# unlikeghost/DeepLearning-MPI

Hardware: AMD Instinct MI355X
Metric: images/sec (whole node) ResNet-50 DDP bs=256/GPU (higher is better)
Workload: dtype bf16; 1 GPU; model=resnet50, global_batch=256, image=224, in_channels=3, per_gpu_batch=256, parallelism=dp1, backend=single, device=cuda, optimizer=SGD(momentum=0.9, wd=1e-5), hipgraph=False

## Files before the change

### deeplearning_mpi_amd/csrc/binding/conv_bwd.cpp

```cpp
#include <c10/hip/HIPCachingAllocator.h>

#include <algorithm>
#include <vector>

#include "common.h"
#include "ops.h"

namespace dlmpi_ext {

using dlmpi::ConvArgs;
using dlmpi::ConvPhase;
using dlmpi::DgradStreamArgs;
using dlmpi::make_fastdiv;
using dlmpi::WgradArgs;

c10::optional<at::Tensor> conv2d_dgrad_pro(const at::Tensor& dy, int N, int P, int Q, int K, int lddy, int dyoff,
                                       const at::Tensor& wT, int C, int R, int S, int stride, int pad, int H, int W,
                                       at::Tensor dx, int lddx, int dxoff, const c10::optional<at::Tensor>& res,
                                       int ldres, int resoff, const c10::optional<at::Tensor>& mask, int ldmask,
                                       int maskoff, const c10::optional<at::Tensor>& z, int ldz, int zoff,
                                       const c10::optional<at::Tensor>& z2, int ldz2, int z2off,
                                       const c10::optional<at::Tensor>& mscale,
                                       const c10::optional<at::Tensor>& mshift,
                                       const c10::optional<at::Tensor>& mbits, bool colsum, int pro,
                                       const c10::optional<at::Tensor>& pk0, const c10::optional<at::Tensor>& pk1,
                                       const c10::optional<at::Tensor>& pz, int ldpz, int pzoff,
                                       const c10::optional<at::Tensor>& bias) {
  require_gpu(dy, "dy");
  if (stride > 2) throw std::runtime_error("conv2d_dgrad: stride <= 2 supported");
  if (bias.has_value() && bias->defined() && (bias->scalar_type() != at::kFloat || bias->numel() < C))
    throw std::runtime_error("conv2d_dgrad: bias must be fp32 [C]");
  ConvArgs a{};
  a.f32 = act_f32(dy, "conv2d_dgrad");
  same_type(dy, wT, "conv2d_dgrad wT");
  same_type(dy, dx, "conv2d_dgrad dx");
  same_type(dy, res, "conv2d_dgrad res");
  same_type(dy, mask, "conv2d_dgrad mask");
  same_type(dy, z, "conv2d_dgrad z");
  same_type(dy, z2, "conv2d_dgrad z2");
  a.x = ptr<uint16_t>(dy);
  a.H = P; a.W = Q; a.C = K; a.ldx = lddy; a.xoff = dyoff;
  a.w = ptr<uint16_t>(wT);
  a.ldw = R * S * K;
  a.S = S;
  a.OH = H; a.OW = W;
  a.so = stride; a.sa = 1;
  a.Nimg = N; a.Kout = C;
  fill_epilogue(a, dx, lddx, dxoff, bias, res, ldres, resoff, c10::nullopt, c10::nullopt, false, c10::nullopt);
  a.vec_store = ((lddx % 8) == 0 && (dxoff % 8) == 0) ? 1 : 0;
  a.mask = optr<uint16_t>(mask);
  a.ldmask = ldmask; a.maskoff = maskoff;
  a.z = optr<uint16_t>(z);
  a.ldz = ldz; a.zoff = zoff;
  a.z2 = optr<uint16_t>(z2);
  a.ldz2 = ldz2; a.z2off = z2off;
  a.mscale = optr<float>(mscale);
  a.mshift = optr<float>(mshift);
  a.mbits = optr<uint8_t>(mbits);
  if (a.mbits && (mbits->numel() != (int64_t)N * H * W * (C / 8) || C % 8))
    throw std::runtime_error("conv2d_dgrad: mask bits must be [N*H*W][C/8]");
  a.nstat = a.z2 ? 3 : 2;
  if (a.z && !a.mask && !a.mscale && !a.mbits)
    throw std::runtime_error("conv2d_dgrad: fused BN statistics need the ReLU mask");
  if (a.mscale && (!a.z || !a.mshift)) throw std::runtime_error("conv2d_dgrad: mask from z needs z, scale, shift");
  if ((a.mask || a.mscale || a.mbits) && ((ldmask | maskoff | ldz | zoff | ldz2 | z2off) % 8 != 0 || !a.vec_store))
    throw std::runtime_error("conv2d_dgrad: fused BN tensors must be 8-channel aligned");
  g_ran.dgrad_stream = 0;
  g_ran.conv3 = 0;
  if (R == 1 && S == 1 && K == 8) g_ran.head_dgrad = 0;
  {
    const int mode = a.mscale ? 2 : 0;
    int th, tw, G;
    if (stream3x3_shape(N, H, W, K, C, R, S, stride, pad, pro, a.f32, th, tw, G) && P == H && Q == W && !colsum &&
        !a.mask && !a.mbits && !a.z2 && !a.res && !a.bias && (a.z != nullptr) == (mode == 2) && a.vec_store &&
        a.kvalid == C && (lddy | dyoff) % 8 == 0 && (int64_t)H * W * lddx * 2 < (1ll << 31) &&
        dx.scalar_type() == at::kBFloat16) {
      dlmpi::Conv3StreamArgs c = conv3_args(dy, N, H, W, lddy, dyoff, wT, 1, a.y, lddx, dxoff, th, tw, G);
      c.z = static_cast<const uint16_t*>(a.z);
      c.ldz = ldz; c.zoff = zoff;
      c.mscale = a.mscale; c.mshift = a.mshift;
      c10::optional<at::Tensor> st;
      if (a.z) {
        st = at::empty({(int64_t)G, 2, (int64_t)C}, dy.options().dtype(at::kFloat));
        c.stats = ptr<float>(*st);
      }
      check(dlmpi_conv3x3_stream(&c, mode == 2 ? 2 : 1, cur_stream()), "conv2d_dgrad (stream 3x3)");
      g_ran.conv3 = 1;
      return st;
    }
  }
  {
    const int64_t M = (int64_t)N * H * W;
    const int mode = a.mbits ? 1 : (a.mscale ? 2 : 0);
    int sbm, sbn, G;
    const auto fits = [](int64_t rows, int64_t ld) { return rows * ld < (1ll << 31); };
    if (R == 1 && S == 1 && stride == 1 && pad == 0 && !a.f32 && pro == 0 && !colsum && !a.mask &&
        (a.z != nullptr) == (mode != 0) && a.vec_store && a.kvalid == C && (lddy | dyoff) % 8 == 0 &&
        (!a.res || (ldres | resoff) % 8 == 0) && fits(M, lddy) && fits(M, lddx) && (!a.res || fits(M, ldres)) &&
        (!a.z || fits(M, ldz)) && (!a.z2 || fits(M, ldz2)) && dx.scalar_type() == at::kBFloat16 &&
        dlmpi_dgrad_stream_plan(M, K, C, mode, a.z2 ? 1 : 0, a.res ? 1 : 0, &sbm, &sbn, &G)) {
      DgradStreamArgs sa{};
      sa.x = ptr<uint16_t>(dy);
      sa.ldx = lddy; sa.xoff = dyoff;
      sa.w = ptr<uint16_t>(wT);
      sa.y = reinterpret_cast<uint16_t*>(a.y);
      sa.ldy = lddx; sa.yoff = dxoff;
      sa.y_bytes = (int)std::min<int64_t>(INT32_MAX, (int64_t)dx.numel() * 2);
      sa.M = (int)M; sa.K = K; sa.Kout = C;
      sa.bias = a.bias;
      sa.res = static_cast<const uint16_t*>(a.res);
      sa.ldres = ldres; sa.resoff = resoff;
      sa.z = static_cast<const uint16_t*>(a.z);
      sa.ldz = ldz; sa.zoff = zoff;
      sa.z2 = static_cast<const uint16_t*>(a.z2);
      sa.ldz2 = ldz2; sa.z2off = z2off;
      sa.mbits = a.mbits;
      sa.mscale = a.mscale; sa.mshift = a.mshift;
      sa.G = G; sa.ntiles = C / sbn; sa.mtiles = (int)ceil_div(M, sbm);
      c10::optional<at::Tensor> st;
      if (a.z) {
        st = at::empty({(int64_t)G, (int64_t)a.nstat, (int64_t)C}, dy.options().dtype(at::kFloat));
        sa.stats = ptr<float>(*st);
// ... 229 lines not shown
  a.ntiles = ceil_div(a.TC, bn);
  const int tiles = a.mtiles * a.ntiles;
  const int target_blocks = g_sw.wgrad_blocks > 0 ? g_sw.wgrad_blocks : 512;
  const int maxsplit = std::max(1, ceil_div(a.npix, 512));
  int splits = std::max(1, std::min(maxsplit, w256 ? target_blocks / tiles : ceil_div(target_blocks, tiles)));
  int pps = ceil_div(a.npix, splits);
  pps = ceil_div(pps, 64) * 64;
  splits = ceil_div(a.npix, pps);
  a.splits = splits;
  a.pix_per_split = pps;
  a.fdPQ = make_fastdiv((uint32_t)(P * Q));
  a.fdQ = make_fastdiv((uint32_t)Q);
  a.fdC = make_fastdiv((uint32_t)C);
  a.fdS = make_fastdiv((uint32_t)S);
  const int64_t wsz = (int64_t)Ko * a.TC;
  const int G = splits > 1 ? dlmpi_wgrad_reduce_groups(splits, wsz) : 0;
  at::Tensor ws = at::empty({(int64_t)(splits + G) * wsz}, dy.options().dtype(at::kFloat));
  a.ws = ptr<float>(ws);
  check(dlmpi_conv_wgrad(&a, bm, bn, cur_stream()), "conv2d_wgrad");
  wgrad_reduce_or_defer(ws, splits, G, wsz, Ko, R * S, C, Creal, Ko_real, grad);
}

void conv2d_wgrad(const at::Tensor& dy, int lddy, int dyoff, int Ko, const at::Tensor& x, int N, int H, int W, int C,
                  int ldx, int xoff, int R, int S, int stride, int pad, int P, int Q, at::Tensor grad, int Creal,
                  int Ko_real) {
  conv2d_wgrad_pro(dy, lddy, dyoff, Ko, x, N, H, W, C, ldx, xoff, R, S, stride, pad, P, Q, grad, Creal, Ko_real, 0,
                   c10::nullopt, c10::nullopt, 0, 0, 0, c10::nullopt, c10::nullopt);
}

void register_conv_bwd(pybind11::module& m) {
  m.def("conv2d_dgrad", &conv2d_dgrad);
  m.def("conv2d_dgrad_pro", &conv2d_dgrad_pro);
  m.def("conv2d_wgrad", &conv2d_wgrad);
  m.def("conv2d_wgrad_pro", &conv2d_wgrad_pro);
  m.def("set_wgrad_defer", [](bool on) {
    if (!on) wgrad_flush();
    g_wgrad_defer = on;
  });
  m.def("wgrad_flush", &wgrad_flush);
  m.def("wgrad_discard", &wgrad_discard);
  m.def("set_wgrad_batch", [](int n) { g_wgrad_batch = n > 0 && n <= dlmpi::kWgradBatch ? n : dlmpi::kWgradBatch; });
  m.def("set_defer_direct", [](int on) { g_defer_direct = on != 0; });
  m.def("set_wgrad_bypass", [](bool on) { g_wgrad_bypass = on; });
  m.def("wgrad_pending", []() { return (int)g_pending.size(); });
  m.def("wgrad_reduce_launches", []() { return g_reduce_launches; });
  m.def("set_dgrad_stream", [](int mode) { dlmpi_set_dgrad_stream(mode); });
  m.def("set_wgrad_fast", [](int on) { dlmpi_set_wgrad_fast(on); });
  def_int(m, "set_conv_pipe_dgrad", nullptr, &g_sw.pipe_dgrad);
  def_int(m, "set_wgrad3", nullptr, &g_sw.wgrad3);
  def_int(m, nullptr, "wgrad3_last", &g_ran.wgrad3);
  def_int(m, "set_wgrad3_blocks", nullptr, &g_sw.wgrad3_blocks);
  def_int(m, "set_wgrad_blocks", nullptr, &g_sw.wgrad_blocks);
  def_int(m, nullptr, "dgrad_stream_last", &g_ran.dgrad_stream);
  def_int(m, nullptr, "head_dgrad_last", &g_ran.head_dgrad);
}

}
```

### deeplearning_mpi_amd/csrc/binding/conv_plan.h

```cpp
#pragma once
#include <cstdint>
#include <vector>

#include "../kernels/dlmpi_kernels.h"

namespace dlmpi_ext {

static inline int ceil_div(int64_t a, int64_t b) { return (int)((a + b - 1) / b); }

struct Switches {
  int pipe = -1;
  int pipe_dgrad = -1;
  int apply = -1;
  int halo = -1;
  int halo_first = 1;
  int splitk = 0;
  int autotune = -1;
  int head = 1;
  int c8 = 1;
  int c16 = 1;
  int c3pro = 1;
  int convT_stream = 1;
  int wgrad3 = -1;
  int wgrad3_blocks = 0;
  int wgrad_blocks = 0;
};
struct LastRan {
  int halo = 0;
  int stream = 0;
  int dgrad_stream = 0;
  int conv3 = 0;
  int head = 0;
  int c8 = 0;
  int c16 = 0;
  int convT_stream = 0;
  int wgrad3 = 0;
  int head_dgrad = 0;
};
extern Switches g_sw;
extern LastRan g_ran;
bool conv_autotune_on();

struct ConvShape {
  int N, H, W, C, K, R, S, stride, pad;
  int pro, f32;
  int bm_req, bn_req;
  int P() const { return (H + 2 * pad - R) / stride + 1; }
  int Q() const { return (W + 2 * pad - S) / stride + 1; }
  int64_t M() const { return (int64_t)N * P() * Q(); }
  int64_t red() const { return (int64_t)R * S * C; }
  bool free_tiles() const { return bm_req <= 0 && bn_req <= 0; }
};

enum class FwdPath { c8, c16, head, stream3x3, stream1x1, apply1x1, pipe, halo, igemm };
const char* fwd_path_name(FwdPath p);

struct FwdOperands {
  bool has_res, has_scale, relu, has_stats, has_fin;
  int kvalid;
  int ldx, xoff, ldy, yoff, ldw;
  int ldpro;
  bool y_bf16, y_f32, w_bf16;
  bool plain(int K) const { return !has_res && !has_scale && !relu && kvalid == K; }
  bool x_aligned() const { return ldx % 8 == 0 && xoff % 8 == 0; }
  bool y_aligned() const { return ldy % 8 == 0 && yoff % 8 == 0; }
};

struct FwdPlan {
  FwdPath path;
  int bm, bn, pipe;
  int rows;
  int G, th, tw, sbm, sbn;
};

void set_kstep(dlmpi::ConvArgs& a, int C);

struct TileQuery {
  int64_t M;
  int Kout;
  int64_t red;
  int cin;
  int R, S, stride, pad, P, Q;
  int f32, pro;
// ... 25 lines not shown
```

### deeplearning_mpi_amd/csrc/kernels/conv_igemm.hip

```cpp
#include <cstdlib>
#include <type_traits>

#include "common.h"

namespace dlmpi {

typedef __attribute__((address_space(3))) void lds_void;

__device__ __forceinline__ void glds16(const void* g, char* lds_wave_base) {
  __builtin_amdgcn_global_load_lds(g, (lds_void*)lds_wave_base, 16, 0, 0);
}

template <int BM, int BN, int NT, int WM>
struct EpiSmem {
  static constexpr int NP0 = BM < 128 ? 1 : (BM / 64 < WM / 16 ? BM / 64 : WM / 16);
  static constexpr int NP = (WM / 16) % NP0 == 0 ? NP0 : WM / 16;
  static constexpr int CS_LD = BN + 4;
  static constexpr int EPI = (BM / NP) * CS_LD * 4;
  static constexpr int RED = (NT / (BN / 8)) * 3 * BN * 4;
  static constexpr int bytes = EPI > RED ? EPI : RED;
};

template <int NT, int NF>
__device__ __forceinline__ bool splitk_combine(const ConvArgs& a, f32x4* acc, char* smem, int tid, int mt, int nt) {
// ... 872 lines not shown
    issue_halo();
    issue_b(0);
  }
  auto step = [&](int ks, auto SLc) {
    constexpr int sl = decltype(SLc)::value;
    asm volatile("s_waitcnt vmcnt(0)\n\ts_waitcnt lgkmcnt(0)" ::: "memory");
    __builtin_amdgcn_s_barrier();
    asm volatile("" ::: "memory");
    int a_addr[TM];
#pragma unroll
    for (int mi = 0; mi < TM; ++mi) {
      const int r = hb[mi] + toff;
      a_addr[mi] = r * 128 + ((fg ^ (r & 7)) << 4);
    }
    const bool more = ks + 1 < nk;
    const bool chunk_end = more && t_cur + 1 == NTAP;
    if (more) tap_next();
#pragma unroll
    for (int kk = 0; kk < 2; ++kk) {
      const int ch = kk * 4 + fg;
      bf16x8 af[TM], bfr[TN];
#pragma unroll
      for (int ni = 0; ni < TN; ++ni)
        bfr[ni] = *reinterpret_cast<const bf16x8*>(smem + b_row0 + sl * B_BYTES + ni * 16 * 128 + ((ch ^ sw) << 4));
#pragma unroll
      for (int mi = 0; mi < TM; ++mi)
        af[mi] = *reinterpret_cast<const bf16x8*>(smem + (kk ? (a_addr[mi] ^ 64) : a_addr[mi]));
      if (kk == 0 && more && !chunk_end) {
        issue_b(sl ^ 1);
        asm volatile("" ::: "memory");
      }
#pragma unroll
      for (int mi = 0; mi < TM; ++mi)
#pragma unroll
        for (int ni = 0; ni < TN; ++ni)
          acc[mi][ni] = __builtin_amdgcn_mfma_f32_16x16x32_bf16(af[mi], bfr[ni], acc[mi][ni], 0, 0, 0);
    }
    if (chunk_end) {
      asm volatile("s_waitcnt lgkmcnt(0)" ::: "memory");
      __builtin_amdgcn_s_barrier();
      asm volatile("" ::: "memory");
      issue_halo();
      issue_b(sl ^ 1);
    }
  };
  for (int ks = 0; ks < nk; ks += 2) {
    step(ks, std::integral_constant<int, 0>{});
    if (ks + 1 < nk) step(ks + 1, std::integral_constant<int, 1>{});
  }
  __syncthreads();
  conv_epilogue<BM, BN, NT, WGM, WGN, uint16_t, true>(a, ph, acc, smem, tid, m0, n0, mt, hn, hh0, hw0);
}

template <int BM, int BN, int WGM, int WGN>
__global__ __launch_bounds__(512) __attribute__((amdgpu_waves_per_eu(BN <= 128 ? 4 : 2, 8)))
void conv1x1_apply_kernel(const ConvArgs a) {
  constexpr int NT = 512;
  static_assert(WGM * WGN == 8, "8 waves");
  constexpr int WM = BM / WGM, WN = BN / WGN, TM = WM / 16, TN = WN / 16;
  constexpr int A_BYTES = BM * 128, B_BYTES = BN * 128, SB = A_BYTES + B_BYTES;
  constexpr int MAXC = 4 * BN;
  constexpr int PRM_BYTES = 4 * MAXC * 4;
  constexpr int EPI_NEED = EpiSmem<BM, BN, NT, WM>::bytes;
  constexpr int SMEM = 2 * SB + PRM_BYTES > EPI_NEED ? 2 * SB + PRM_BYTES : EPI_NEED;
  constexpr int RP = NT / 8;
  constexpr int AL = BM / RP, BL = BN / RP;
  static_assert(AL >= 1 && BL >= 1, "tile shape");
  __shared__ __attribute__((aligned(16))) char smem[SMEM];

  const int tid = threadIdx.x, lane = tid & 63;
  const int wid = __builtin_amdgcn_readfirstlane(tid >> 6);
  const int wm = wid / WGN, wn = wid % WGN;
  const int lrow = tid >> 3, jc = tid & 7;
  const ConvPhase& ph = a.ph[0];
  const int M = a.Nimg * ph.P * ph.Q;
  const uint32_t mt = xcd_remap(blockIdx.x, (uint32_t)ph.mtiles);
  const int m0 = (int)mt * BM;
  const int C = a.C, nk = C / 64;
  const bool rbn = a.prscale != nullptr;

  float* prm = reinterpret_cast<float*>(smem + 2 * SB);
  for (int i = tid; i < C; i += NT) {
    prm[i] = a.pscale[i];
    prm[MAXC + i] = a.pshift[i];
    if (rbn) {
      prm[2 * MAXC + i] = a.prscale[i];
      prm[3 * MAXC + i] = a.prshift[i];
    }
  }

  const uint16_t* xb = static_cast<const uint16_t*>(a.x);
  const uint16_t* rb = static_cast<const uint16_t*>(a.pz);
  uint32_t zo[AL], ro[AL], yo[AL], bo[AL];
  uint32_t okm = 0;
#pragma unroll
  for (int i = 0; i < AL; ++i) {
    const int m = m0 + lrow + RP * i;
    if (m < M) okm |= 1u << i;
    const uint32_t mm = m < M ? (uint32_t)m : 0u;
    zo[i] = mm * (uint32_t)a.ldx + (uint32_t)a.xoff + 8 * jc;
    ro[i] = mm * (uint32_t)a.ldpz + (uint32_t)a.pzoff + 8 * jc;
    yo[i] = mm * (uint32_t)a.ldpy + (uint32_t)a.pyoff + 8 * jc;
    bo[i] = mm * (uint32_t)(C >> 3) + jc;
  }
  const uint16_t* wb = static_cast<const uint16_t*>(a.w) + (int64_t)lrow * a.ldw + 8 * jc;
  const int64_t wstep = (int64_t)RP * a.ldw;

  u32x4 zv[AL], rv[AL], wv[BL];
  auto load = [&](int k) {
    const int c = 64 * k;
#pragma unroll
    for (int i = 0; i < AL; ++i) {
      zv[i] = *reinterpret_cast<const u32x4*>(xb + zo[i] + c);
      rv[i] = *reinterpret_cast<const u32x4*>(rb + ro[i] + c);
    }
#pragma unroll
    for (int i = 0; i < BL; ++i) wv[i] = *reinterpret_cast<const u32x4*>(wb + i * wstep + c);
  };
  auto commit = [&](int k, int buf) {
    char* As = smem + buf * SB;
    char* Bs = As + A_BYTES;
    const int cc = 64 * k + 8 * jc;
    const f32x4 s0 = *reinterpret_cast<const f32x4*>(prm + cc), s1 = *reinterpret_cast<const f32x4*>(prm + cc + 4);
    const f32x4 h0 = *reinterpret_cast<const f32x4*>(prm + MAXC + cc);
    const f32x4 h1 = *reinterpret_cast<const f32x4*>(prm + MAXC + cc + 4);
#pragma unroll
    for (int i = 0; i < AL; ++i) {
      const int r = lrow + RP * i;
      u32x4 pk = u32x4{0u, 0u, 0u, 0u};
      if ((okm >> i) & 1) {
        float v[8], q[8];
        unpack8(zv[i], v);
        unpack8(rv[i], q);
#pragma unroll
        for (int e = 0; e < 4; ++e) {
          v[e] = __builtin_fmaf(v[e], s0[e], h0[e]);
          v[e + 4] = __builtin_fmaf(v[e + 4], s1[e], h1[e]);
        }
        if (rbn) {
          const f32x4 a0 = *reinterpret_cast<const f32x4*>(prm + 2 * MAXC + cc);
          const f32x4 a1 = *reinterpret_cast<const f32x4*>(prm + 2 * MAXC + cc + 4);
          const f32x4 b0 = *reinterpret_cast<const f32x4*>(prm + 3 * MAXC + cc);
          const f32x4 b1 = *reinterpret_cast<const f32x4*>(prm + 3 * MAXC + cc + 4);
#pragma unroll
          for (int e = 0; e < 4; ++e) {
            q[e] = __builtin_fmaf(q[e], a0[e], b0[e]);
            q[e + 4] = __builtin_fmaf(q[e + 4], a1[e], b1[e]);
          }
        }
#pragma unroll
        for (int e = 0; e < 8; ++e) v[e] = fmaxf(v[e] + q[e], 0.f);
        pk = pack8(v);
        *reinterpret_cast<u32x4*>(a.py + yo[i] + 64 * k) = pk;
        uint32_t b = 0;
#pragma unroll
        for (int t = 0; t < 4; ++t) {
          b |= (uint32_t)((pk[t] & 0xffffu) != 0u && !(pk[t] & 0x8000u)) << (2 * t);
          b |= (uint32_t)((pk[t] >> 16) != 0u && !(pk[t] & 0x80000000u)) << (2 * t + 1);
        }
        a.pmbits[bo[i] + 8 * k] = (uint8_t)b;
      }
      *reinterpret_cast<u32x4*>(As + r * 128 + ((jc ^ (r & 7)) << 4)) = pk;
    }
#pragma unroll
    for (int i = 0; i < BL; ++i) {
      const int r = lrow + RP * i;
      *reinterpret_cast<u32x4*>(Bs + r * 128 + ((jc ^ (r & 7)) << 4)) = wv[i];
    }
  };

  f32x4 acc[TM][TN];
#pragma unroll
  for (int mi = 0; mi < TM; ++mi)
#pragma unroll
    for (int ni = 0; ni < TN; ++ni) acc[mi][ni] = f32x4{0.f, 0.f, 0.f, 0.f};
  const int fr = lane & 15, fg = lane >> 4;

  load(0);
  __syncthreads();
  commit(0, 0);
  __syncthreads();
  for (int k = 0; k < nk; ++k) {
    if (k + 1 < nk) load(k + 1);
// ... 47 lines not shown
  return S < 2 ? 1 : S;
}

static hipError_t launch_f32(const ConvArgs* a, int bm, int bn, dim3 grid, hipStream_t s) {
  if (a->pro != 0) return hipErrorInvalidValue;
  const bool small = a->C < 32 || a->C % 32 != 0;
#define LAUNCH_F32(BM_, BN_)                                                                                   \
  do {                                                                                                       \
    if (small) hipLaunchKernelGGL((conv_igemm_kernel<BM_, BN_, true, 2, 0, float>), grid, dim3(256), 0, s, *a); \
    else hipLaunchKernelGGL((conv_igemm_kernel<BM_, BN_, false, 2, 0, float>), grid, dim3(256), 0, s, *a);     \
  } while (0)
  if (bm == 128 && bn == 128) LAUNCH_F32(128, 128);
  else if (bm == 128 && bn == 64) LAUNCH_F32(128, 64);
  else if (bm == 64 && bn == 128) LAUNCH_F32(64, 128);
  else if (bm == 64 && bn == 64) LAUNCH_F32(64, 64);
  else return hipErrorInvalidValue;
#undef LAUNCH_F32
  return hipGetLastError();
}

static hipError_t launch_pipe(const ConvArgs* a, int bm, int bn, int var, dim3 grid, hipStream_t s) {
  if (a->f32 || a->pro != 0 || a->C % 64 != 0 || a->C > kPipeMaxC || a->halo || grid.y != 1) return hipErrorInvalidValue;
  if (var != (bm == 128 ? 4 : 2)) return hipErrorInvalidValue;
  if (bm == 256 && bn == 256) hipLaunchKernelGGL((conv_pipe_kernel<256, 256, 2, 4, 2, 2>), grid, dim3(512), 0, s, *a);
  else if (bm == 224 && bn == 256) hipLaunchKernelGGL((conv_pipe_kernel<224, 256, 2, 4, 2, 2>), grid, dim3(512), 0, s, *a);
  else if (bm == 256 && bn == 128) hipLaunchKernelGGL((conv_pipe_kernel<256, 128, 4, 2, 3, 2>), grid, dim3(512), 0, s, *a);
  else if (bm == 128 && bn == 256) hipLaunchKernelGGL((conv_pipe_kernel<128, 256, 2, 4, 3, 4>), grid, dim3(512), 0, s, *a);
  else if (bm == 512 && bn == 64) hipLaunchKernelGGL((conv_pipe_kernel<512, 64, 8, 1, 2, 2>), grid, dim3(512), 0, s, *a);
  else return hipErrorInvalidValue;
  return hipGetLastError();
}

extern "C" int dlmpi_conv1x1_apply_ok(int C, int K) {
  return C % 64 == 0 && C <= 4 * K && (K == 64 || K == 128 || K == 256);
}

extern "C" hipError_t dlmpi_conv1x1_apply(const ConvArgs* a, int bm, hipStream_t s) {
  if (a->pro != 3 || a->f32 || a->halo || a->nphase != 1 || a->ntiles != 1 || !a->vec_store || a->res ||
      a->scale || a->relu || a->mask || a->mscale || a->mbits || a->z || a->splitk_req > 1 ||
      !dlmpi_conv1x1_apply_ok(a->C, a->Kout) || a->ph[0].Tr != 1 || a->ph[0].Ts != 1 || a->sa != 1 ||
      a->ph[0].mtiles != (a->Nimg * a->ph[0].P * a->ph[0].Q + bm - 1) / bm || a->ldw != a->C ||
      (int64_t)a->Nimg * a->H * a->W * (a->ldx > a->ldpz ? (a->ldx > a->ldpy ? a->ldx : a->ldpy)
                                                          : (a->ldpz > a->ldpy ? a->ldpz : a->ldpy)) >= (1ll << 31))
    return hipErrorInvalidValue;
  const dim3 grid((unsigned)a->ph[0].mtiles);
  if (grid.x == 0) return hipSuccess;
  if (bm == 128 && a->Kout == 64) hipLaunchKernelGGL((conv1x1_apply_kernel<128, 64, 8, 1>), grid, dim3(512), 0, s, *a);
  else if (bm == 128 && a->Kout == 128) hipLaunchKernelGGL((conv1x1_apply_kernel<128, 128, 4, 2>), grid, dim3(512), 0, s, *a);
  else if (bm == 128 && a->Kout == 256) hipLaunchKernelGGL((conv1x1_apply_kernel<128, 256, 2, 4>), grid, dim3(512), 0, s, *a);
  else return hipErrorInvalidValue;
  return hipGetLastError();
}

static int g_halo_pipe = 1;
extern "C" void dlmpi_set_halo_pipe(int on) { g_halo_pipe = on; }

extern "C" hipError_t dlmpi_conv_igemm_ex(const ConvArgs* a_in, int bm, int bn, int pipe, hipStream_t s) {
  int maxt = 0, tiles = 0, maxk = 0;
  for (int i = 0; i < a_in->nphase; ++i) {
    maxt = a_in->ph[i].mtiles > maxt ? a_in->ph[i].mtiles : maxt;
    tiles += a_in->ph[i].mtiles * a_in->ntiles;
    maxk = a_in->ph[i].ksteps > maxk ? a_in->ph[i].ksteps : maxk;
  }
  ConvArgs ab = *a_in;
  const ConvArgs* a = &ab;
  ab.splitk = 1;
  if (pipe) {
    const dim3 grid((unsigned)(maxt * a->ntiles), 1, (unsigned)a->nphase);
    if (grid.x == 0) return hipSuccess;
    return launch_pipe(a, bm, bn, pipe - 1, grid, s);
  }
  int S = a_in->splitk_req > 0 ? a_in->splitk_req : splitk_plan(tiles, maxk);
  if (S > maxk) S = maxk > 0 ? maxk : 1;
  if (S > 1) {
    const int ntile_ids = maxt * a_in->ntiles * a_in->nphase;
    float* slab = dlmpi_splitk_slab(s, (size_t)ntile_ids * S * bm * bn);
    int* tk = dlmpi_splitk_tickets(s, ntile_ids);
    if (slab && tk) {
      ab.splitk = S;
      ab.sk_slab = slab;
      ab.sk_tk = tk;
    }
  }
  dim3 grid((unsigned)(maxt * a->ntiles), (unsigned)ab.splitk, (unsigned)a->nphase);
  if (grid.x == 0) return hipSuccess;
  if (a->f32) return launch_f32(a, bm, bn, grid, s);
  if (a->halo) {
    if (a->pro != 0 || a->C % 64 != 0) return hipErrorInvalidValue;
    if (bm == 128 && bn == 128) hipLaunchKernelGGL((conv_igemm_kernel<128, 128, false, 2, 0, uint16_t, true>), grid, dim3(256), 0, s, *a);
    else if (bm == 128 && bn == 64) hipLaunchKernelGGL((conv_igemm_kernel<128, 64, false, 2, 0, uint16_t, true>), grid, dim3(256), 0, s, *a);
    else if (bm == 256 && bn == 64) hipLaunchKernelGGL((conv_igemm_kernel<256, 64, false, 4, 0, uint16_t, true>), grid, dim3(256), 0, s, *a);
    else if (bm == 256 && bn == 128) {
      if (g_halo_pipe && ab.splitk == 1) hipLaunchKernelGGL((conv_halo_pipe_kernel<256, 128, 2>), grid, dim3(256), 0, s, *a);
      else hipLaunchKernelGGL((conv_igemm_kernel<256, 128, false, 2, 0, uint16_t, true>), grid, dim3(256), 0, s, *a);
    } else return hipErrorInvalidValue;
    return hipGetLastError();
  }
  if (a->pro != 0 && (a->pro != 3 || a->C < 64 || a->C % 64 != 0)) return hipErrorInvalidValue;
  hipError_t e = hipSuccess;
  if (bm == 256 && bn == 64) {
    if (a->pro == 3) return hipErrorInvalidValue;
    if (a->C < 64) hipLaunchKernelGGL((conv_igemm_kernel<256, 64, true, 4>), grid, dim3(256), 0, s, *a);
    else hipLaunchKernelGGL((conv_igemm_kernel<256, 64, false, 4>), grid, dim3(256), 0, s, *a);
  } else if (bm == 256 && bn == 128) e = launch_tile<256, 128>(a, grid, s);
  else if (bm == 128 && bn == 128) e = launch_tile<128, 128>(a, grid, s);
  else if (bm == 128 && bn == 64) e = launch_tile<128, 64>(a, grid, s);
// ... 10 lines not shown
```

### deeplearning_mpi_amd/csrc/kernels/dlmpi_kernels.h

```cpp
#pragma once
#include <hip/hip_runtime_api.h>
#include <stdint.h>

namespace dlmpi {

struct FastDiv {
  uint32_t d, mul, shr;
};
inline FastDiv make_fastdiv(uint32_t d) {
  FastDiv f;
  f.d = d;
  uint32_t l = 0;
  while ((1ull << l) < d) ++l;
  f.mul = (uint32_t)((((1ull << 32) * ((1ull << l) - d)) / d) + 1);
  f.shr = l;
  return f;
}

struct FinArgs {
  int mode;
  double count;
  const float* gamma;
  const float* beta;
  float* running_mean;
// ... 143 lines not shown
  const uint16_t* w;
  int ldw, flip;
  uint16_t* y;
  int ldy, yoff;
  int N, H, W;
  int th, tw, tiles_h, tiles_w, ntiles, G;
  const float* bias;
  const uint16_t* z;
  int ldz, zoff;
  const float* mscale;
  const float* mshift;
  float* stats;
  const float* psc;
  const float* psh;
  uint16_t* py;
  int ldpy, pyoff;
};

struct WgradReduceEntry {
  const float* ws;
  float* ws2;
  float* out;
  int64_t total;
  int splits, G, Ko_real, T, Cpad, Creal;
  int block1;
  int block2;
};
constexpr int kWgradBatch = 16;
struct WgradReduceBatch {
  int n;
  WgradReduceEntry e[kWgradBatch];
};

struct Wgrad3Args {
  const void* dy;
  int ldy, dyoff, Ko;
  const void* x;
  int ldx, xoff, C;
  int H, W;
  int tiles_h, tiles_w, ntiles_pix, tiles_per_split;
  int mtiles, ntiles, splits;
  float* ws;
};

}

extern "C" {
void dlmpi_set_wgrad_fast(int on);
void dlmpi_set_halo_pipe(int on);
hipError_t dlmpi_conv_igemm(const dlmpi::ConvArgs* a, int bm, int bn, hipStream_t s);
hipError_t dlmpi_conv_igemm_ex(const dlmpi::ConvArgs* a, int bm, int bn, int pipe, hipStream_t s);
int dlmpi_conv1x1_apply_ok(int C, int K);
hipError_t dlmpi_conv1x1_apply(const dlmpi::ConvArgs* a, int bm, hipStream_t s);
hipError_t dlmpi_conv_wgrad(const dlmpi::WgradArgs* a, int bm, int bn, hipStream_t s);
int dlmpi_wgrad_pro_ok(int direct, int pro_a, int pro_b);
hipError_t dlmpi_wgrad_reduce(const float* ws, int splits, int Ko, int T, int Cpad, int Creal,
                              int Ko_real, float* out, float* ws2, int ws2_floats, hipStream_t s);
int dlmpi_wgrad_reduce_groups(int splits, int64_t total);
hipError_t dlmpi_wgrad_reduce_batch(dlmpi::WgradReduceBatch* b, hipStream_t s);
int dlmpi_wgrad3_plan(int Ko, int C, int* kt, int* ct);
hipError_t dlmpi_wgrad3x3(const dlmpi::Wgrad3Args* a, int kt, int ct, hipStream_t s);
int dlmpi_head1x1_ok(int C, int kv);
int dlmpi_conv3x3_c8_blocks(int64_t pixels);
int dlmpi_conv4x4_c16_blocks(int64_t pixels);
hipError_t dlmpi_conv4x4_c16(const void* x, int ldx, int xoff, int N, int U, int V, const void* w, const float* bias,
                             void* y, int ldy, int yoff, float* stats, int G, hipStream_t s);
hipError_t dlmpi_conv3x3_c8(const void* x, int ldx, int xoff, int N, int H, int W, const void* w, const float* bias,
                            void* y, int ldy, int yoff, float* stats, int G, hipStream_t s);
hipError_t dlmpi_head1x1(const void* x, int ldx, int xoff, int64_t M, int C, const void* w, int ldw,
                         const float* bias, void* y, int ldy, int yoff, int kv, int y_f32, const float* psc,
                         const float* psh, hipStream_t s);
int dlmpi_conv3_stream_plan(int N, int H, int W, int C, int K, int blocks, int* th, int* tw, int* G);
hipError_t dlmpi_conv3x3_stream(const dlmpi::Conv3StreamArgs* a, int mode, hipStream_t s);
void dlmpi_set_conv3_stream(int mode);

hipError_t dlmpi_bn_finalize(const float* partial, int ntiles, int C, double count, const float* gamma,
                             const float* beta, float* running_mean, float* running_var, float momentum,
                             float eps, float* scale, float* shift, float* save_mean, float* save_invstd,
                             double* ws, hipStream_t s);
int dlmpi_colsum_ws_doubles(int T, int C);
hipError_t dlmpi_set_aux_stream(hipStream_t s, int role);
hipError_t dlmpi_bn_stats(const void* x, int64_t M, int C, int ldx, int xoff, float* partial, int nblk, int f32,
                          hipStream_t s);
hipError_t dlmpi_bn_apply(const void* x, int ldx, int xoff, int64_t M, int C, const float* scale, const float* shift,
                          const void* res, int ldres, int resoff, int relu, void* y, int ldy, int yoff, uint8_t* mbits,
                          int f32, hipStream_t s);
hipError_t dlmpi_bn_apply2(const void* x, int ldx, int xoff, int64_t M, int C, const float* scale, const float* shift,
                           const void* res, int ldres, int resoff, const float* rscale, const float* rshift, int relu,
                           void* y, int ldy, int yoff, uint8_t* mbits, int f32, hipStream_t s);
hipError_t dlmpi_bn_bwd_reduce(const void* dy, int lddy, int dyoff, const void* ymask, int ldym, int ymoff,
                               const void* x, int ldx, int xoff, int64_t M, int C, const float* mean,
                               const float* invstd, float* partial, int nblk, int f32, hipStream_t s);
hipError_t dlmpi_bn_bwd_finalize(const float* partial, int nblk, int C, double count, const float* gamma,
                                 const float* mean, const float* invstd, float* dgamma, float* dbeta,
                                 float* coef, double* ws, hipStream_t s);
hipError_t dlmpi_bn_bwd_finalize_ex(const float* partial, int nblk, int ns, int k2, int raw_z, int C, double count,
                                    const float* gamma, const float* mean, const float* invstd, float* dgamma,
                                    float* dbeta, float* coef, double* ws, hipStream_t s);
hipError_t dlmpi_bn_bwd_apply(const void* dy, int lddy, int dyoff, const void* ymask, int ldym, int ymoff,
                              const void* x, int ldx, int xoff, int64_t M, int C, const float* coef, void* dx,
                              void* dyr_out, int f32, hipStream_t s);
hipError_t dlmpi_dual_dgrad_weights(const void* w, int C, int K, const float* coef, void* w2, float* b, int f32,
                                    hipStream_t s);
hipError_t dlmpi_channel_sum(const void* x, int64_t M, int C, int ldx, int xoff, float* out_acc, float* partial,
                             int nblk, double* ws, int f32, hipStream_t s);
int dlmpi_reduce_blocks(int64_t M, int C);
// ... 102 lines not shown
```

### deeplearning_mpi_amd/models/engine.py

```python
from __future__ import annotations

import contextlib
import os
from typing import NamedTuple, Optional

import torch
import torch.nn as nn

from ..ops.act import Act, Deferred, padc
from ..ops.backend import make_backend
from ..utils.arena import ParamArena
from ..utils.profiler import range as trace_range


@contextlib.contextmanager
def grad_side(be, *tensors):
    side = getattr(be, "side_stream", None)
    if side is None:
        yield
        return
    cur = torch.cuda.current_stream()
    side.wait_stream(cur)
    torch.cuda.set_stream(side)
    try:
        yield
    finally:
        torch.cuda.set_stream(cur)
    if _STREAM_HOLD:
        be.held.extend(t for t in tensors if t is not None)
        return
    for t in tensors:
        if t is not None:
            t.record_stream(side)


def record_on(stream, *objs):
    if _STREAM_HOLD:
        return
    for o in objs:
        if o is None:
            continue
        if isinstance(o, torch.Tensor):
            if o.is_cuda:
                o.record_stream(stream)
        elif isinstance(o, Deferred):
            record_on(stream, *o.bufs())
        elif hasattr(o, "buf") and isinstance(getattr(o, "buf"), torch.Tensor):
            record_on(stream, o.buf)
        elif isinstance(o, (tuple, list)):
            record_on(stream, *o)


_STREAM_HOLD = True

_OUTER_DGRAD = True
_HEAD_DGRAD = True

DEFER_BN_WGRAD = True

DUAL_DGRAD = True
DUAL_MIN_ROWS = 2 * 256 * 28 * 28
DUAL_WGRAD_PRO = True

FUSE_APPLY = True
FUSE_APPLY_MAX_K = 256
FUSE_APPLY_3X3 = True

WGRAD_TAIL_MAIN = True


def img_rows(a, n0: int, n1: int):
    if a is None:
        return None
    if isinstance(a, Deferred):
        return Deferred(a.kind, img_rows(a.src, n0, n1), img_rows(a.z, n0, n1), a.k0, a.k1)
    hw = a.H * a.W
    return Act(a.buf[n0 * hw:n1 * hw], n1 - n0, a.H, a.W, a.C, a.off)


class PendingApply:

    __slots__ = ("y", "z", "scale", "shift", "res", "relu", "mbits", "done")

    def __init__(self, y, z, scale, shift, res, relu, mbits):
        self.y, self.z, self.scale, self.shift, self.res, self.relu, self.mbits = y, z, scale, shift, res, relu, mbits
        self.done = False

    N = property(lambda self: self.y.N)
    H = property(lambda self: self.y.H)
    W = property(lambda self: self.y.W)
    C = property(lambda self: self.y.C)
    device = property(lambda self: self.y.device)

    def resolve(self, be) -> Act:
        if not self.done:
            be.bn_apply(self.z, self.scale, self.shift, self.res, self.relu, self.y, mbits=self.mbits)
            self.done = True
        return self.y


def resolve(be, a):
    return a.resolve(be) if isinstance(a, PendingApply) else a


def bufs(*objs):
    out = []
    for o in objs:
        if o is None:
            continue
        if isinstance(o, Deferred):
            out.extend(o.bufs())
        elif isinstance(o, Act):
            out.append(o.buf)
        else:
            out.append(o)
    return out


class BwdFuse(NamedTuple):
# ... 168 lines not shown
        if before_res is not None and res is not None:
            before_res()
        invstd = torch.rsqrt(bn.running_var + bn.eps)
        scale = bn.weight.data * invstd if bn.affine else invstd
        shift = (bn.bias.data if bn.affine else 0.0) - bn.running_mean * scale
        if self.bias is not None:
            shift = shift + self.bias.data * scale
        be.conv_fwd(x, wf, self.Kp, self.R, self.S, self.stride, self.pad, y, res=res, scale=scale.contiguous(),
                    shift=shift.contiguous(), relu=self.relu)
        return y, None

    @staticmethod
    def fuse_spec(ctx, z2=None) -> BwdFuse:
        x, z, y, mean, invstd, scale, shift, has_res, mbits = ctx
        if has_res or z2 is not None:
            return BwdFuse(None if mbits is not None else y, z, z2, mbits=mbits)
        return BwdFuse(None, z, None, scale, shift)

    def bwd(self, be, ctx, dy: Act, need_dx=True, dx_res: Act = None, dyr_out: Act = None, ymask: Act = None,
            use_own_mask=True, pre=None, k2=1, fuse_next=None, colsum=False, before_res=None, dx_out: Act = None):
        ar = self.arena
        bn = self.bn
        dg_in, dg_w, dg_b = None, None, None
        if bn is not None and need_dx and pre is not None and dyr_out is None and self.dual:
            x, z = ctx[0], ctx[1]
            if (z.off == z.C and z.ld == 2 * z.C and dy.off == 0 and dy.ld == z.ld
                    and dy.buf.data_ptr() == z.buf.data_ptr()):
                mean, invstd = ctx[3], ctx[4]
                gam = bn.weight.data if bn.affine else None
                dzd = be.bn_bwd_deferred(dy, z, mean, invstd, gam, ar.grad_flat(bn.weight) if bn.affine else None,
                                         ar.grad_flat(bn.bias) if bn.affine else None, pre=pre, k2=k2)
                with grad_side(be, *bufs(dzd, x)):
                    if bn.affine:
                        ar.ready(bn.weight, bn.bias)
                    if self.bias is not None:
                        ar.ready(self.bias)
                    self._wgrad(be, dzd if (DUAL_WGRAD_PRO and getattr(be, "prologue", False)) else be.materialize(dzd), x)
                    ar.ready(self.conv.weight)
                dg_w, dg_b = be.dual_weights(ar.get_compute(self.h_dg), self.Cp, self.Kp, dzd.k0)
                dg_in = Act(z.buf, z.N, z.H, z.W, 2 * z.C)
                bn = None
        if dg_in is not None:
            x = ctx[0]
        elif bn is not None:
            x, z, y, mean, invstd = ctx[:5]
            if pre is not None:
                mask = None
            else:
                mask = ymask if ymask is not None else (y if (self.relu and use_own_mask) else None)
            gam = bn.weight.data if bn.affine else None
            dgam = ar.grad_flat(bn.weight) if bn.affine else None
            dbet = ar.grad_flat(bn.bias) if bn.affine else None
            defer = not need_dx and DEFER_BN_WGRAD and getattr(be, "prologue", False)
            if pre is not None and mask is None and dyr_out is None and defer:
                dz = be.bn_bwd_deferred(dy, z, mean, invstd, gam, dgam, dbet, pre=pre, k2=k2)
            else:
                dz = Act.empty(z.N, z.H, z.W, z.C, be.act_dtype, z.device)
                be.bn_bwd(dy, mask, z, mean, invstd, gam, dgam, dbet, dz, dyr_out, pre=pre, k2=k2)
            if self.wgrad_main and WGRAD_TAIL_MAIN and not need_dx:
                self._wgrad(be, dz, x)
                with grad_side(be, *bufs(dz, x)):
                    if bn.affine:
                        ar.ready(bn.weight, bn.bias)
                    if self.bias is not None:
                        ar.ready(self.bias)
                    ar.ready(self.conv.weight)
            else:
                with grad_side(be, *bufs(dz, x)):
                    if bn.affine:
                        ar.ready(bn.weight, bn.bias)
                    if self.bias is not None:
                        ar.ready(self.bias)
                    self._wgrad(be, dz, x)
                    ar.ready(self.conv.weight)
        else:
            x, y = ctx
            assert not self.relu, "ReLU without BN is not used by the engine models"
            dz = dy
            with grad_side(be, *bufs(dz, x)):
                if self.bias is not None:
                    if self.Kp == self.K:
                        be.channel_sum(dz, ar.grad_flat(self.bias))
                    else:
                        tmp = torch.empty(self.Kp, dtype=be.dt, device=dz.device)
                        be.fill_(tmp, 0.0)
                        be.channel_sum(dz, tmp)
                        if getattr(self, "_kidx", None) is None or self._kidx.device != dz.device:
                            self._kidx = torch.arange(self.K, device=dz.device)
                        be.gather_(ar.grad_flat(self.bias), tmp, self._kidx, accumulate=True)
                    ar.ready(self.bias)
                self._wgrad(be, dz, x)
                ar.ready(self.conv.weight)
        if not need_dx:
            return None
        if before_res is not None:
            before_res()
        if dx_out is not None:
            assert (dx_out.N, dx_out.H, dx_out.W, dx_out.C) == (x.N, x.H, x.W, self.Cp), (dx_out, x, self.Cp)
            dx = dx_out
        else:
            dx = Act.empty(x.N, x.H, x.W, self.Cp, be.act_dtype, x.device)
        if dg_in is not None:
            part = be.conv_dgrad(dg_in, dg_w, self.Cp, 1, 1, 1, 0, dx, res=dx_res, fuse=fuse_next, colsum=colsum,
                                 bias=dg_b)
            return (dx, part) if (fuse_next is not None or colsum) else dx
        if (self.K == 1 and self.R == 1 and self.S == 1 and self.stride == 1 and dx_res is None and not colsum
# ... 256 lines not shown
```

### deeplearning_mpi_amd/ops/backend.py

```python
from __future__ import annotations

import os
import weakref
import struct

import torch
import torch.nn.functional as F

from .act import Act, Deferred


_AUX_STREAMS = {}
_BACKENDS = weakref.WeakSet()


def _new_aux_stream(idx, C, role):
    with torch.cuda.device(idx):
        st = torch.cuda.ExternalStream(C.create_stream(), device=torch.device("cuda", idx))
        C.set_aux_stream(st.cuda_stream, role)
    return st


def _aux_stream(device, C, role):
    idx = device.index if device.index is not None else torch.cuda.current_device()
# ... 116 lines not shown
                                 res.ld if res is not None else 0, res.off if res is not None else 0, scale, shift,
                                 bool(relu), stats, 0, int(kvalid), 0)

    def conv_fwd_bn(self, x, w, K, R, S, stride, pad, z: Act, bias, stats, count, gamma, beta, rm, rv, momentum,
                    eps, scale, shift, save_mean, save_invstd):
        x = self.materialize(x)
        self.C.conv2d_fwd_bn(x.buf, x.N, x.H, x.W, x.C, x.ld, x.off, w, K, R, S, stride, pad, z.buf, z.ld, z.off,
                             bias, stats, 0, None, None, None, 0, 0, float(count), gamma, beta, rm, rv,
                             float(momentum), float(eps), scale, shift, save_mean, save_invstd)

    def conv_fwd_bn_apply(self, xp, w, K, z: Act, bias, stats, count, gamma, beta, rm, rv, momentum, eps, scale,
                          shift, save_mean, save_invstd):
        x, res = xp.z, xp.res
        rs = rh = None
        if isinstance(res, Deferred):
            assert res.kind == "bn", res
            res, rs, rh = res.src, res.k0, res.k1
        y = xp.y
        self.C.conv2d_fwd_bn_apply(x.buf, x.N, x.H, x.W, x.C, x.ld, x.off, w, K, z.buf, z.ld, z.off, bias, stats,
                                   xp.scale, xp.shift, res.buf, res.ld, res.off, rs, rh, y.buf, y.ld, y.off, xp.mbits,
                                   float(count), gamma, beta, rm, rv, float(momentum), float(eps), scale, shift,
                                   save_mean, save_invstd)

    def conv3_pro_ok(self, z: Act, y: Act) -> bool:
        return bool(self.C.conv3_pro_ok(z.N, z.H, z.W, z.C, 64, z.ld, z.off, y.ld, y.off, y.ld, y.off))

    def conv3_fwd_bn_apply(self, xp, w, K, z: Act, bias, stats, count, gamma, beta, rm, rv, momentum, eps, scale,
                           shift, save_mean, save_invstd):
        x, y = xp.z, xp.y
        r = self.C.conv3x3_fwd_bn_apply(x.buf, x.N, x.H, x.W, x.ld, x.off, w, z.buf, z.ld, z.off, bias, stats,
                                        xp.scale, xp.shift, y.buf, y.ld, y.off, float(count), gamma, beta, rm, rv,
                                        float(momentum), float(eps), scale, shift, save_mean, save_invstd)
        if r < 0:
            self.bn_apply(xp.z, xp.scale, xp.shift, None, True, y)
            self.conv_fwd_bn(y, w, K, 3, 3, 1, 1, z, bias, stats, count, gamma, beta, rm, rv, momentum, eps, scale,
                             shift, save_mean, save_invstd)

    def conv_fwd_bnbwd(self, x: Act, w, K, R, S, stride, pad, y: Act, fuse):
        z = fuse.z
        return self.C.conv2d_fwd_bnbwd(x.buf, x.N, x.H, x.W, x.C, x.ld, x.off, w, K, R, S, stride, pad, y.buf, y.ld,
                                       y.off, z.buf, z.ld, z.off, fuse.scale, fuse.shift)

    def conv_dgrad(self, dy: Act, wT, C, R, S, stride, pad, dx: Act, res: Act = None, fuse=None, colsum=False,
                   bias=None):
        m, z, z2, sc, sh, mb = fuse if fuse is not None else (None, None, None, None, None, None)

        def t(a):
            return (a.buf, a.ld, a.off) if a is not None else (None, 0, 0)

        dy = self.materialize(dy)
        return self.C.conv2d_dgrad_pro(dy.buf, dy.N, dy.H, dy.W, dy.C, dy.ld, dy.off, wT, C, R, S, stride, pad, dx.H,
                                       dx.W, dx.buf, dx.ld, dx.off, *t(res), *t(m), *t(z), *t(z2), sc, sh, mb,
                                       bool(colsum and fuse is None), 0, None, None, None, 0, 0, bias)

    def dual_weights(self, wT, C, K, coef):
        w2 = torch.empty(C, 2 * K, dtype=self.act_dtype, device=self.device)
        b = torch.empty(C, dtype=torch.float32, device=self.device)
        self.C.dual_dgrad_weights(wT, C, K, coef, w2, b)
        return w2, b

    def convT_fwd(self, x: Act, wf, Cout, y: Act, bias=None):
        self.C.convT2x2_fwd(x.buf, x.N, x.H, x.W, x.C, x.ld, x.off, wf, Cout, y.buf, y.ld, y.off, bias)

    def wgrad_defer(self, on: bool):
        self.C.set_wgrad_defer(bool(on))

    def wgrad_flush(self):
        self.C.wgrad_flush()

    def wgrad_discard(self):
        self.C.wgrad_discard()

    def wgrad_bypass(self, on: bool):
        self.C.set_wgrad_bypass(bool(on))

    def conv_wgrad(self, dy, x, R, S, stride, pad, grad, Creal, Ko_real):
        direct = R == 1 and S == 1 and stride == 1 and pad == 0
        if isinstance(dy, Deferred) and isinstance(x, Deferred) or (isinstance(x, Deferred) and not direct):
            x = self.materialize(x)
        dy, pa, ca, _, zb, zld, zoff = self._pro(dy)
        x, pb, sb, hb, _, _, _ = self._pro(x)
        assert pa in (0, 2) and pb in (0, 1)
        self.C.conv2d_wgrad_pro(dy.buf, dy.ld, dy.off, dy.C, x.buf, x.N, x.H, x.W, x.C, x.ld, x.off, R, S, stride,
                                pad, dy.H, dy.W, grad, Creal, Ko_real, pa, ca, zb, zld, zoff, pb, sb, hb)

    def bn_finalize(self, stats, ntiles, C, count, gamma, beta, rm, rv, momentum, eps, scale, shift, save_mean,
                    save_invstd):
        self.C.bn_finalize(stats, ntiles, C, float(count), gamma, beta, rm, rv, float(momentum), float(eps), scale,
                           shift, save_mean, save_invstd)

    def bn_stats(self, x: Act):
        nblk = self.C.reduce_blocks(x.rows, x.C)
        part = torch.empty(nblk, 2, x.C, dtype=torch.float32, device=x.device)
        self.C.bn_stats(x.buf, x.rows, x.C, x.ld, x.off, part, nblk)
        return part, nblk

    def bn_apply(self, x: Act, scale, shift, res, relu, y: Act, mbits=None):
        rs = rh = None
        if isinstance(res, Deferred):
            assert res.kind == "bn", res
            res, rs, rh = res.src, res.k0, res.k1
        self.C.bn_apply(x.buf, x.ld, x.off, x.rows, x.C, scale, shift, res.buf if res is not None else None,
                        res.ld if res is not None else 0, res.off if res is not None else 0, bool(relu), y.buf, y.ld,
                        y.off, mbits, rs, rh)

    def bn_bwd_deferred(self, dy: Act, x: Act, mean, invstd, gamma, dgamma, dbeta, pre, k2=1) -> Deferred:
# ... 632 lines not shown
```

Baseline: 13440 images/sec.

## Fuse BN-backward apply into the 1x1 convolution dgrad prologue

```diff
diff --git a/deeplearning_mpi_amd/csrc/binding/conv_bwd.cpp b/deeplearning_mpi_amd/csrc/binding/conv_bwd.cpp
--- a/deeplearning_mpi_amd/csrc/binding/conv_bwd.cpp
+++ b/deeplearning_mpi_amd/csrc/binding/conv_bwd.cpp
@@ -67,7 +67,54 @@
     throw std::runtime_error("conv2d_dgrad: fused BN tensors must be 8-channel aligned");
   g_ran.dgrad_stream = 0;
   g_ran.conv3 = 0;
+  g_ran.dgrad_bnbwd = 0;
   if (R == 1 && S == 1 && K == 8) g_ran.head_dgrad = 0;
+  if (pro == 4) {
+    const int64_t M = (int64_t)N * H * W;
+    const auto holds = [M](const at::Tensor& t, int ld, int off, int ch) {
+      return M == 0 || t.numel() >= (M - 1) * ld + off + ch;
+    };
+    if (!pk0.has_value() || !pk0->defined() || pk0->scalar_type() != at::kFloat || pk0->numel() < 3 * (int64_t)K ||
+        !pz.has_value() || !pz->defined() || K % 8 || !holds(*pz, ldpz, pzoff, K) || !holds(dy, lddy, dyoff, K))
+      throw std::runtime_error("conv2d_dgrad: prologue 4 needs fp32 coef [3][K] and the BN input z [M][K]");
+    same_type(dy, pz, "conv2d_dgrad pz");
+    same_type(dy, pk1, "conv2d_dgrad dz");
+    const bool store = pk1.has_value() && pk1->defined();
+    if (store && pk1->numel() < M * K) throw std::runtime_error("conv2d_dgrad: dz must be [M][K]");
+    const bool fused =
+        g_sw.bnbwd != 0 && !a.f32 && R == 1 && S == 1 && stride == 1 && pad == 0 && P == H && Q == W && !colsum &&
+        !a.res && !a.mask && !a.mbits && !a.z2 && a.vec_store && a.kvalid == C && dx.scalar_type() == at::kBFloat16 &&
+        (lddy | dyoff | ldpz | pzoff) % 8 == 0 && (!a.z || (ldz | zoff) % 8 == 0) && (a.z != nullptr) == (a.mscale != nullptr) &&
+        dlmpi_conv1x1_bnbwd_dgrad_ok(K, C) && M * std::max(std::max(lddy, ldpz), std::max(lddx, std::max(ldz, K))) < (1ll << 31) &&
+        wT.numel() >= (int64_t)C * K && holds(dx, lddx, dxoff, C) && (!a.z || holds(*z, ldz, zoff, C)) &&
+        (!a.mscale || (mscale->numel() >= C && mshift->numel() >= C));
+    if (!fused) {
+      at::Tensor dz = store ? *pk1 : at::empty({M, (int64_t)K}, dy.options());
+      check(dlmpi_bn_bwd_apply(dy.data_ptr(), lddy, dyoff, nullptr, 0, 0, pz->data_ptr(), ldpz, pzoff, M, K,
+                               ptr<float>(*pk0), dz.data_ptr(), nullptr, a.f32, cur_stream()),
+            "conv2d_dgrad (bn_bwd_apply)");
+      return conv2d_dgrad_pro(dz, N, P, Q, K, K, 0, wT, C, R, S, stride, pad, H, W, dx, lddx, dxoff, res, ldres, resoff,
+                              mask, ldmask, maskoff, z, ldz, zoff, z2, ldz2, z2off, mscale, mshift, mbits, colsum, 0,
+                              c10::nullopt, c10::nullopt, c10::nullopt, 0, 0, bias);
+    }
+    constexpr int bm = 128;
+    a.pro = 4;
+    a.pscale = ptr<float>(*pk0);
+    a.pz = ptr<uint16_t>(*pz);
+    a.ldpz = ldpz; a.pzoff = pzoff;
+    a.py = store ? ptr<uint16_t>(*pk1) : nullptr;
+    a.ldpy = K; a.pyoff = 0;
+    a.ntiles = 1;
+    single_phase(a, H, W, 1, 1, 0, bm);
+    c10::optional<at::Tensor> st;
+    if (a.z) {
+      st = at::empty({(int64_t)a.ph[0].mtiles, 2, (int64_t)C}, dy.options().dtype(at::kFloat));
+      a.stats = ptr<float>(*st);
+    }
+    check(dlmpi_conv1x1_bnbwd_dgrad(&a, bm, cur_stream()), "conv2d_dgrad (fused BN-backward apply 1x1)");
+    g_ran.dgrad_bnbwd = 1;
+    return st;
+  }
   {
     const int mode = a.mscale ? 2 : 0;
     int th, tw, G;
@@ -403,6 +450,9 @@
   def_int(m, "set_wgrad3_blocks", nullptr, &g_sw.wgrad3_blocks);
   def_int(m, "set_wgrad_blocks", nullptr, &g_sw.wgrad_blocks);
   def_int(m, nullptr, "dgrad_stream_last", &g_ran.dgrad_stream);
+  def_int(m, "set_dgrad_bnbwd", nullptr, &g_sw.bnbwd);
+  def_int(m, nullptr, "dgrad_bnbwd_last", &g_ran.dgrad_bnbwd);
+  m.def("dgrad_bnbwd_ok", [](int K, int C) { return g_sw.bnbwd != 0 && dlmpi_conv1x1_bnbwd_dgrad_ok(K, C) != 0; });
   def_int(m, nullptr, "head_dgrad_last", &g_ran.head_dgrad);
 }
 
diff --git a/deeplearning_mpi_amd/csrc/binding/conv_plan.h b/deeplearning_mpi_amd/csrc/binding/conv_plan.h
--- a/deeplearning_mpi_amd/csrc/binding/conv_plan.h
+++ b/deeplearning_mpi_amd/csrc/binding/conv_plan.h
@@ -12,6 +12,7 @@
   int pipe = -1;
   int pipe_dgrad = -1;
   int apply = -1;
+  int bnbwd = -1;
   int halo = -1;
   int halo_first = 1;
   int splitk = 0;
@@ -29,6 +30,7 @@
   int halo = 0;
   int stream = 0;
   int dgrad_stream = 0;
+  int dgrad_bnbwd = 0;
   int conv3 = 0;
   int head = 0;
   int c8 = 0;
diff --git a/deeplearning_mpi_amd/csrc/kernels/conv_igemm.hip b/deeplearning_mpi_amd/csrc/kernels/conv_igemm.hip
--- a/deeplearning_mpi_amd/csrc/kernels/conv_igemm.hip
+++ b/deeplearning_mpi_amd/csrc/kernels/conv_igemm.hip
@@ -948,7 +948,7 @@
   conv_epilogue<BM, BN, NT, WGM, WGN, uint16_t, true>(a, ph, acc, smem, tid, m0, n0, mt, hn, hh0, hw0);
 }
 
-template <int BM, int BN, int WGM, int WGN>
+template <int BM, int BN, int WGM, int WGN, int XF = 0>
 __global__ __launch_bounds__(512) __attribute__((amdgpu_waves_per_eu(BN <= 128 ? 4 : 2, 8)))
 void conv1x1_apply_kernel(const ConvArgs a) {
   constexpr int NT = 512;
@@ -973,15 +973,21 @@
   const uint32_t mt = xcd_remap(blockIdx.x, (uint32_t)ph.mtiles);
   const int m0 = (int)mt * BM;
   const int C = a.C, nk = C / 64;
-  const bool rbn = a.prscale != nullptr;
+  const bool rbn = XF == 0 && a.prscale != nullptr;
 
   float* prm = reinterpret_cast<float*>(smem + 2 * SB);
   for (int i = tid; i < C; i += NT) {
-    prm[i] = a.pscale[i];
-    prm[MAXC + i] = a.pshift[i];
-    if (rbn) {
-      prm[2 * MAXC + i] = a.prscale[i];
-      prm[3 * MAXC + i] = a.prshift[i];
+    if constexpr (XF == 1) {
+      prm[i] = a.pscale[i];
+      prm[MAXC + i] = a.pscale[C + i];
+      prm[2 * MAXC + i] = a.pscale[2 * C + i];
+    } else {
+      prm[i] = a.pscale[i];
+      prm[MAXC + i] = a.pshift[i];
+      if (rbn) {
+        prm[2 * MAXC + i] = a.prscale[i];
+        prm[3 * MAXC + i] = a.prshift[i];
+      }
     }
   }
 
@@ -1024,7 +1030,22 @@
     for (int i = 0; i < AL; ++i) {
       const int r = lrow + RP * i;
       u32x4 pk = u32x4{0u, 0u, 0u, 0u};
-      if ((okm >> i) & 1) {
+      if constexpr (XF == 1) {
+        if ((okm >> i) & 1) {
+          const f32x4 t0 = *reinterpret_cast<const f32x4*>(prm + 2 * MAXC + cc);
+          const f32x4 t1 = *reinterpret_cast<const f32x4*>(prm + 2 * MAXC + cc + 4);
+          float g[8], q[8];
+          unpack8(zv[i], g);
+          unpack8(rv[i], q);
+#pragma unroll
+          for (int e = 0; e < 4; ++e) {
+            g[e] = __builtin_fmaf(s0[e], g[e], __builtin_fmaf(h0[e], q[e], t0[e]));
+            g[e + 4] = __builtin_fmaf(s1[e], g[e + 4], __builtin_fmaf(h1[e], q[e + 4], t1[e]));
+          }
+          pk = pack8(g);
+          if (a.py) *reinterpret_cast<u32x4*>(a.py + yo[i] + 64 * k) = pk;
+        }
+      } else if ((okm >> i) & 1) {
         float v[8], q[8];
         unpack8(zv[i], v);
         unpack8(rv[i], q);
@@ -1178,6 +1199,30 @@
   return hipGetLastError();
 }
 
+extern "C" int dlmpi_conv1x1_bnbwd_dgrad_ok(int C, int K) {
+  return C >= 64 && C % 64 == 0 && C <= 4 * K && (K == 128 || K == 256);
+}
+
+extern "C" hipError_t dlmpi_conv1x1_bnbwd_dgrad(const ConvArgs* a, int bm, hipStream_t s) {
+  const int ldmax = std::max(std::max(a->ldx, a->ldpz), a->py ? a->ldpy : 0);
+  if (a->pro != 4 || a->f32 || a->out_f32 || a->halo || a->nphase != 1 || a->ntiles != 1 || !a->vec_store || a->res ||
+      a->scale || a->relu || a->mask || a->mbits || a->z2 || a->splitk_req > 1 || !a->x || !a->pz || !a->pscale ||
+      (a->mscale != nullptr) != (a->z != nullptr) || (a->mscale != nullptr) != (a->mshift != nullptr) ||
+      (a->stats != nullptr && !a->z) || !dlmpi_conv1x1_bnbwd_dgrad_ok(a->C, a->Kout) || a->ph[0].Tr != 1 ||
+      a->ph[0].Ts != 1 || a->sa != 1 || a->so != 1 || a->ph[0].P != a->OH || a->ph[0].Q != a->OW ||
+      a->ph[0].mtiles != (a->Nimg * a->ph[0].P * a->ph[0].Q + bm - 1) / bm || a->ldw != a->C ||
+      (a->ldx | a->xoff | a->ldpz | a->pzoff | a->ldy | a->yoff | a->ldz | a->zoff) % 8 != 0 ||
+      (a->py && (a->ldpy | a->pyoff) % 8 != 0) || a->ldx < a->C || a->ldpz < a->C || (a->py && a->ldpy < a->C) ||
+      (int64_t)a->Nimg * a->H * a->W * ldmax >= (1ll << 31))
+    return hipErrorInvalidValue;
+  const dim3 grid((unsigned)a->ph[0].mtiles);
+  if (grid.x == 0) return hipSuccess;
+  if (bm == 128 && a->Kout == 128) hipLaunchKernelGGL((conv1x1_apply_kernel<128, 128, 4, 2, 1>), grid, dim3(512), 0, s, *a);
+  else if (bm == 128 && a->Kout == 256) hipLaunchKernelGGL((conv1x1_apply_kernel<128, 256, 2, 4, 1>), grid, dim3(512), 0, s, *a);
+  else return hipErrorInvalidValue;
+  return hipGetLastError();
+}
+
 static int g_halo_pipe = 1;
 extern "C" void dlmpi_set_halo_pipe(int on) { g_halo_pipe = on; }
 
diff --git a/deeplearning_mpi_amd/csrc/kernels/dlmpi_kernels.h b/deeplearning_mpi_amd/csrc/kernels/dlmpi_kernels.h
--- a/deeplearning_mpi_amd/csrc/kernels/dlmpi_kernels.h
+++ b/deeplearning_mpi_amd/csrc/kernels/dlmpi_kernels.h
@@ -219,6 +219,8 @@
 hipError_t dlmpi_conv_igemm_ex(const dlmpi::ConvArgs* a, int bm, int bn, int pipe, hipStream_t s);
 int dlmpi_conv1x1_apply_ok(int C, int K);
 hipError_t dlmpi_conv1x1_apply(const dlmpi::ConvArgs* a, int bm, hipStream_t s);
+int dlmpi_conv1x1_bnbwd_dgrad_ok(int C, int K);
+hipError_t dlmpi_conv1x1_bnbwd_dgrad(const dlmpi::ConvArgs* a, int bm, hipStream_t s);
 hipError_t dlmpi_conv_wgrad(const dlmpi::WgradArgs* a, int bm, int bn, hipStream_t s);
 int dlmpi_wgrad_pro_ok(int direct, int pro_a, int pro_b);
 hipError_t dlmpi_wgrad_reduce(const float* ws, int splits, int Ko, int T, int Cpad, int Creal,
diff --git a/deeplearning_mpi_amd/models/engine.py b/deeplearning_mpi_amd/models/engine.py
--- a/deeplearning_mpi_amd/models/engine.py
+++ b/deeplearning_mpi_amd/models/engine.py
@@ -65,6 +65,9 @@
 FUSE_APPLY = True
 FUSE_APPLY_MAX_K = 256
 FUSE_APPLY_3X3 = True
+
+FUSE_BNBWD_DGRAD = int(os.environ.get("DLMPI_FUSE_BNBWD_DGRAD", "2"))
+FUSE_BNBWD_MAX_BYTES = int(os.environ.get("DLMPI_FUSE_BNBWD_MAX_MB", "64")) << 20
 
 WGRAD_TAIL_MAIN = True
 
@@ -339,6 +342,36 @@
             dgam = ar.grad_flat(bn.weight) if bn.affine else None
             dbet = ar.grad_flat(bn.bias) if bn.affine else None
             defer = not need_dx and DEFER_BN_WGRAD and getattr(be, "prologue", False)
+            if (FUSE_BNBWD_DGRAD and pre is not None and mask is None and dyr_out is None and need_dx
+                    and self.R == 1 and self.S == 1 and self.stride == 1 and self.pad == 0 and dx_res is None
+                    and not colsum and (fuse_next is None or (fuse_next.scale is not None and fuse_next.z2 is None))
+                    and hasattr(be, "conv_dgrad_bnbwd") and 2 * z.rows * z.C <= FUSE_BNBWD_MAX_BYTES
+                    and be.dgrad_bnbwd_ok(dy, z, self.Cp, dx_out, fuse_next)):
+                dzd = be.bn_bwd_deferred(dy, z, mean, invstd, gam, dgam, dbet, pre=pre, k2=k2)
+                if before_res is not None:
+                    before_res()
+                if dx_out is not None:
+                    assert (dx_out.N, dx_out.H, dx_out.W, dx_out.C) == (x.N, x.H, x.W, self.Cp), (dx_out, x, self.Cp)
+                dx = dx_out if dx_out is not None else Act.empty(x.N, x.H, x.W, self.Cp, be.act_dtype, x.device)
+                store = FUSE_BNBWD_DGRAD != 2
+                dz = Act.empty(z.N, z.H, z.W, z.C, be.act_dtype, z.device) if store else dzd
+
+                def side():
+                    with grad_side(be, *bufs(dz, x)):
+                        if bn.affine:
+                            ar.ready(bn.weight, bn.bias)
+                        if self.bias is not None:
+                            ar.ready(self.bias)
+                        self._wgrad(be, dz, x)
+                        ar.ready(self.conv.weight)
+
+                if not store:
+                    side()
+                part = be.conv_dgrad_bnbwd(dzd, ar.get_compute(self.h_dg), self.Cp, dx, fuse=fuse_next,
+                                           dz=dz if store else None)
+                if store:
+                    side()
+                return (dx, part) if fuse_next is not None else dx
             if pre is not None and mask is None and dyr_out is None and defer:
                 dz = be.bn_bwd_deferred(dy, z, mean, invstd, gam, dgam, dbet, pre=pre, k2=k2)
             else:
diff --git a/deeplearning_mpi_amd/ops/backend.py b/deeplearning_mpi_amd/ops/backend.py
--- a/deeplearning_mpi_amd/ops/backend.py
+++ b/deeplearning_mpi_amd/ops/backend.py
@@ -192,6 +192,28 @@
         return self.C.conv2d_dgrad_pro(dy.buf, dy.N, dy.H, dy.W, dy.C, dy.ld, dy.off, wT, C, R, S, stride, pad, dx.H,
                                        dx.W, dx.buf, dx.ld, dx.off, *t(res), *t(m), *t(z), *t(z2), sc, sh, mb,
                                        bool(colsum and fuse is None), 0, None, None, None, 0, 0, bias)
+
+    def dgrad_bnbwd_ok(self, dy: Act, z: Act, C, dx: Act = None, fuse=None) -> bool:
+        if self.f32 or (dy.ld | dy.off | z.ld | z.off) % 8:
+            return False
+        if dx is not None and (dx.ld | dx.off) % 8:
+            return False
+        if fuse is not None and (fuse.scale is None or fuse.z2 is not None or fuse.mask is not None
+                                 or fuse.mbits is not None or (fuse.z.ld | fuse.z.off) % 8):
+            return False
+        return bool(self.C.dgrad_bnbwd_ok(dy.C, C))
+
+    def conv_dgrad_bnbwd(self, dzd, wT, C, dx: Act, fuse=None, dz: Act = None, res: Act = None):
+        m, z, z2, sc, sh, mb = fuse if fuse is not None else (None, None, None, None, None, None)
+
+        def t(a):
+            return (a.buf, a.ld, a.off) if a is not None else (None, 0, 0)
+
+        dy, bz = dzd.src, dzd.z
+        assert dz is None or (dz.ld == dy.C and dz.off == 0 and dz.rows == dy.rows)
+        return self.C.conv2d_dgrad_pro(dy.buf, dy.N, dy.H, dy.W, dy.C, dy.ld, dy.off, wT, C, 1, 1, 1, 0, dx.H, dx.W,
+                                       dx.buf, dx.ld, dx.off, *t(res), *t(m), *t(z), *t(z2), sc, sh, mb, False, 4,
+                                       dzd.k0, dz.buf if dz is not None else None, bz.buf, bz.ld, bz.off, None)
 
     def dual_weights(self, wT, C, K, coef):
         w2 = torch.empty(C, 2 * K, dtype=self.act_dtype, device=self.device)
```

Result: no change. 13430 images/sec (-0.0%).
